# feiyeha/EGM-Unet

Hardware: AMD Instinct MI355X
Metric: train images/sec at 3x512x512 bs=8/GPU (higher is better)
Workload: dtype bf16; 1 GPU; EGM-UNet GRFBUNet(3,2,base_c=32) fwd+5-term-loss+bwd+SGD, 8x3x512x512 per GPU (BASELINE.json configs[1]); global_batch=8, parallelism=dp1, launch=hipGraph replay, world_size=1

## Files before the change

egm_unet_amd/csrc/mca.hip:

```cpp
#include "common.h"
#include "bn_elem.h"
#include <stdlib.h>

namespace {

inline int stream_grid(long long total_threads) {
    long long b = (total_threads + 255) / 256;
    if (b > 256 * 16) b = 256 * 16;
    if (b < 1) b = 1;
    return (int)b;
}
__device__ __forceinline__ float sigm(float v) { return 1.f / (1.f + expf(-v)); }

template <typename T, int MODE>
__global__ __launch_bounds__(256) void mca_reduce_row_kernel(const T* __restrict__ a, int lda, const T* __restrict__ b, int ldb,
                                                             float* __restrict__ sums, float* __restrict__ colp, float* __restrict__ chp,
                                                             int H, int W, int C, const float* __restrict__ scale = nullptr,
                                                             const float* __restrict__ shift = nullptr, int act = 0,
                                                             T* __restrict__ zout = nullptr, int ldz = 0) {
    __shared__ float st[2 * 256 * 8];
    __shared__ float red[16];
    const int n = blockIdx.y, h = blockIdx.x, tid = threadIdx.x, ncv = C >> 3, slots = 256 / ncv;
    const int cv = tid % ncv, slot = tid / ncv, L = H + W + C;
    const long long rowbase = ((long long)n * H + h) * W;
// ... 214 lines not shown
            for (int q = -1; q <= 1; ++q) {
                if (yy + r < 0 || yy + r >= H || xx + q < 0 || xx + q >= W) continue;
                load8(xo + (p + (long long)r * W + q) * ld + cv * 8, v);
#pragma unroll
                for (int j = 0; j < 8; ++j) {
                    if (v[j] > mx[j]) { mx[j] = v[j]; amx[j] = (r + 1) * 3 + (q + 1); }
                    if (v[j] < mn[j]) { mn[j] = v[j]; amn[j] = (r + 1) * 3 + (q + 1); }
                    s[j] += v[j];
                }
            }
        float o1[8], o2[8];
#pragma unroll
        for (int j = 0; j < 8; ++j) {
            const float sh = to_f32(xo[p * ld + shuffle_src(cv * 8 + j, C)]);
            o1[j] = 0.51f * c[j] + 0.2f * (mx[j] - mn[j]) + 0.1f * sh;
            const float u = c[j] - s[j] * (1.f / 9.f);
            o2[j] = u * u;
        }
        store8(r1 + p * ldr + cv * 8, o1); store8(u2 + p * ldu + cv * 8, o2);
        if (codes != nullptr) {
            uint2 cd;
            cd.x = (amx[0] | (amn[0] << 4)) | ((amx[1] | (amn[1] << 4)) << 8) | ((amx[2] | (amn[2] << 4)) << 16) | ((amx[3] | (amn[3] << 4)) << 24);
            cd.y = (amx[4] | (amn[4] << 4)) | ((amx[5] | (amn[5] << 4)) << 8) | ((amx[6] | (amn[6] << 4)) << 16) | ((amx[7] | (amn[7] << 4)) << 24);
            *reinterpret_cast<uint2*>(codes + p * C + cv * 8) = cd;
        }
    }
}
template <typename T>
__global__ void add_avg3_kernel(const T* __restrict__ a, int lda, const T* __restrict__ b, int ldb, float scale, T* __restrict__ out, int ldo,
                                int N, int H, int W, int C) {
    const int ncv = C >> 3;
    const long long total = (long long)N * H * W * ncv;
    for (long long i = blockIdx.x * 256LL + threadIdx.x; i < total; i += (long long)gridDim.x * 256) {
        long long p; int cv; egm_divmod(i, ncv, p, cv);
        int xx, yy; egm_pix_yx(p, H, W, yy, xx);
        float c[8], s[8], v[8];
        load8(a + p * lda + cv * 8, c);
        zero8(s);
#pragma unroll
        for (int r = -1; r <= 1; ++r)
#pragma unroll
            for (int q = -1; q <= 1; ++q) {
                if (yy + r < 0 || yy + r >= H || xx + q < 0 || xx + q >= W) continue;
                load8(b + (p + (long long)r * W + q) * ldb + cv * 8, v);
#pragma unroll
                for (int j = 0; j < 8; ++j) s[j] += v[j];
            }
#pragma unroll
        for (int j = 0; j < 8; ++j) c[j] += scale * s[j] * (1.f / 9.f);
        store8(out + p * ldo + cv * 8, c);
    }
}
constexpr int MF_TY = 16, MF_TX = 16, MF_CB = 32, MF_PY = MF_TY + 4, MF_PX = MF_TX + 4, MF_UY = MF_TY + 2, MF_UX = MF_TX + 2;
template <typename T>
__global__ __launch_bounds__(256) void mca_fused_fwd_kernel(const T* __restrict__ x, int ldx, const float* __restrict__ gates,
                                                            T* __restrict__ xo, int ldxo, T* __restrict__ out, int ldo,
                                                            unsigned char* __restrict__ codes, int N, int H, int W, int C, int tiles_x,
                                                            int tiles_y, int nchunk, float inv) {
    extern __shared__ __attribute__((aligned(16))) unsigned char mf_smem[];
    T* sxo = reinterpret_cast<T*>(mf_smem);
    T* su2 = sxo + MF_PY * MF_PX * MF_CB;
    const int tid = threadIdx.x, L = H + W + C;
    int b = xcd_contiguous_item(blockIdx.x, gridDim.x);
    const int chunk = b % nchunk; b /= nchunk;
    const int tx = b % tiles_x; b /= tiles_x;
    const int ty = b % tiles_y; const int n = b / tiles_y;
    const int y0 = ty * MF_TY, x0 = tx * MF_TX, c0 = chunk * MF_CB;
    const int nvec = (C - c0 < MF_CB ? C - c0 : MF_CB) >> 3;
    const float* __restrict__ g = gates + (long long)n * L;
    const long long img = (long long)n * H * W;
    __shared__ float sgh[MF_PY], sgw[MF_PX];
    if (tid < MF_PY) { const int gy = y0 + tid - 2; sgh[tid] = (gy >= 0 && gy < H) ? g[gy] : 0.f; }
    else if (tid >= 64 && tid < 64 + MF_PX) { const int gx = x0 + tid - 64 - 2; sgw[tid - 64] = (gx >= 0 && gx < W) ? g[H + gx] : 0.f; }
    const int vt = tid & 3;
    float gc8[8], gs8[8];
#pragma unroll
    for (int j = 0; j < 8; ++j) {
        const bool okv = vt < nvec;
        gc8[j] = okv ? g[H + W + c0 + vt * 8 + j] : 0.f;
        gs8[j] = okv ? g[H + W + shuffle_src(c0 + vt * 8 + j, C)] : 0.f;
    }

    constexpr int NC = MF_TY * MF_TX * 4 / 256;
    T shv[NC][8];
#pragma unroll
    for (int k = 0; k < NC; ++k) {
        const int i = tid + k * 256, pix = i >> 2, v = i & 3, ly = pix / MF_TX, lx = pix - ly * MF_TX;
        const int gy = y0 + ly, gx = x0 + lx;
        const bool ok = v < nvec && gy < H && gx < W;
        const long long p = img + (long long)(ok ? gy : 0) * W + (ok ? gx : 0);
        const int q0 = ok ? ((c0 + v * 8) >> 2) : 0;
#pragma unroll
        for (int grp = 0; grp < 4; ++grp) {
            const T* sp = x + p * ldx + (ok ? grp * (C >> 2) : 0) + q0;
            if (sizeof(T) == 2 && ((C >> 2) & 1) == 0) {
                const uint32_t two = *reinterpret_cast<const uint32_t*>(sp);
                __builtin_memcpy(&shv[k][grp], &two, 2);
                const uint16_t hi = (uint16_t)(two >> 16);
                __builtin_memcpy(&shv[k][grp + 4], &hi, 2);
            } else {
                shv[k][grp] = sp[0]; shv[k][grp + 4] = sp[1];
            }
        }
    }
    constexpr int NA = (MF_PY * MF_PX * 4 + 255) / 256;
    uint4 raw[NA];
#pragma unroll
    for (int k = 0; k < NA; ++k) {
        const int i = tid + k * 256, pix = i >> 2, v = i & 3, py = pix / MF_PX, px = pix - py * MF_PX;
        const int gy = y0 + py - 2, gx = x0 + px - 2;
        raw[k] = make_uint4(0, 0, 0, 0);
        if (i < MF_PY * MF_PX * 4 && v < nvec && gy >= 0 && gy < H && gx >= 0 && gx < W) {
            const T* src = x + (img + (long long)gy * W + gx) * ldx + c0 + v * 8;
            if (sizeof(T) == 2) raw[k] = *reinterpret_cast<const uint4*>(src);
        }
    }
    __syncthreads();
#pragma unroll
    for (int k = 0; k < NA; ++k) {
        const int i = tid + k * 256, pix = i >> 2, v = i & 3, py = pix / MF_PX, px = pix - py * MF_PX;
        const int gy = y0 + py - 2, gx = x0 + px - 2;
        if (i >= MF_PY * MF_PX * 4) continue;
        float val[8];
        zero8(val);
        if (v < nvec && gy >= 0 && gy < H && gx >= 0 && gx < W) {
            const long long p = img + (long long)gy * W + gx;
            if (sizeof(T) == 2) load8(reinterpret_cast<const T*>(&raw[k]), val);
            else load8(x + p * ldx + c0 + v * 8, val);
            const float ghw = sgh[py] + sgw[px];
#pragma unroll
            for (int j = 0; j < 8; ++j) val[j] = to_f32(from_f32<T>(val[j] * ((ghw + gc8[j]) * inv)));
            if (xo != nullptr && py >= 2 && py < MF_TY + 2 && px >= 2 && px < MF_TX + 2) store8(xo + p * ldxo + c0 + v * 8, val);
        }
        store8_lds(sxo + pix * MF_CB + v * 8, val);
    }
    __syncthreads();
    for (int i = tid; i < MF_UY * MF_UX * 4; i += 256) {
        const int pix = i >> 2, v = i & 3, uy = pix / MF_UX, ux = pix - uy * MF_UX;
        const int gy = y0 + uy - 1, gx = x0 + ux - 1;
        float o2[8];
        zero8(o2);
        if (v < nvec && gy >= 0 && gy < H && gx >= 0 && gx < W) {
            float c[8], s8[8], t[8];
            zero8(s8);
            const T* ctr = sxo + ((uy + 1) * MF_PX + ux + 1) * MF_CB + v * 8;
            load8(ctr, c);
#pragma unroll
            for (int r = -1; r <= 1; ++r)
#pragma unroll
                for (int q = -1; q <= 1; ++q) {
                    load8(ctr + (r * MF_PX + q) * MF_CB, t);
#pragma unroll
                    for (int j = 0; j < 8; ++j) s8[j] += t[j];
                }
#pragma unroll
            for (int j = 0; j < 8; ++j) { const float u = c[j] - s8[j] * (1.f / 9.f); o2[j] = u * u; }
        }
        store8_lds(su2 + pix * MF_CB + v * 8, o2);
    }
    __syncthreads();
#pragma unroll
    for (int k = 0; k < NC; ++k) {
        const int i = tid + k * 256;
        const int pix = i >> 2, v = i & 3, ly = pix / MF_TX, lx = pix - ly * MF_TX;
        const int gy = y0 + ly, gx = x0 + lx;
        if (v >= nvec || gy >= H || gx >= W) continue;
        const long long p = img + (long long)gy * W + gx;
        float c[8], mx[8], mn[8], t[8], s2[8];
        int amx[8], amn[8];
        const T* ctr = sxo + ((ly + 2) * MF_PX + lx + 2) * MF_CB + v * 8;
        const T* uctr = su2 + ((ly + 1) * MF_UX + lx + 1) * MF_CB + v * 8;
        load8(ctr, c);
        zero8(s2);
#pragma unroll
        for (int j = 0; j < 8; ++j) { mx[j] = -INFINITY; mn[j] = INFINITY; amx[j] = 4; amn[j] = 4; }
#pragma unroll
        for (int r = -1; r <= 1; ++r)
#pragma unroll
            for (int q = -1; q <= 1; ++q) {
                load8(uctr + (r * MF_UX + q) * MF_CB, t);
#pragma unroll
                for (int j = 0; j < 8; ++j) s2[j] += t[j];
                if (gy + r < 0 || gy + r >= H || gx + q < 0 || gx + q >= W) continue;
                load8(ctr + (r * MF_PX + q) * MF_CB, t);
#pragma unroll
                for (int j = 0; j < 8; ++j) {
                    if (t[j] > mx[j]) { mx[j] = t[j]; amx[j] = (r + 1) * 3 + (q + 1); }
                    if (t[j] < mn[j]) { mn[j] = t[j]; amn[j] = (r + 1) * 3 + (q + 1); }
                }
            }
        const float ghw = sgh[ly + 2] + sgw[lx + 2];
        float o[8];
#pragma unroll
        for (int j = 0; j < 8; ++j) {
            const float sh = to_f32(from_f32<T>(to_f32(shv[k][j]) * ((ghw + gs8[j]) * inv)));
            const float o1 = to_f32(from_f32<T>(0.51f * c[j] + 0.2f * (mx[j] - mn[j]) + 0.1f * sh));
            o[j] = o1 + 0.2f * s2[j] * (1.f / 9.f);
        }
        store8(out + p * ldo + c0 + v * 8, o);
        if (codes != nullptr) {
            uint2 cd;
            cd.x = (amx[0] | (amn[0] << 4)) | ((amx[1] | (amn[1] << 4)) << 8) | ((amx[2] | (amn[2] << 4)) << 16) | ((amx[3] | (amn[3] << 4)) << 24);
            cd.y = (amx[4] | (amn[4] << 4)) | ((amx[5] | (amn[5] << 4)) << 8) | ((amx[6] | (amn[6] << 4)) << 16) | ((amx[7] | (amn[7] << 4)) << 24);
            *reinterpret_cast<uint2*>(codes + p * C + c0 + v * 8) = cd;
        }
    }
}
template <typename T>
__global__ void mca_bwd_du_kernel(const T* __restrict__ xo, int ld, const T* __restrict__ g, int ldg, T* __restrict__ du, int ldd, int N, int H,
                                  int W, int C) {
    const int ncv = C >> 3;
    const long long total = (long long)N * H * W * ncv;
    for (long long i = blockIdx.x * 256LL + threadIdx.x; i < total; i += (long long)gridDim.x * 256) {
// ... 134 lines not shown
        const T* gctr = sg + ((ly + 2) * MB_P + lx + 2) * MB_CB + v * 8;
        const unsigned char* cctr = scd + ((ly + 1) * MB_U + lx + 1) * MB_CB + v * 8;
#pragma unroll
        for (int r = -1; r <= 1; ++r)
#pragma unroll
            for (int q = -1; q <= 1; ++q) {
                load8(dctr + (r * MB_U + q) * MB_CB, t);
#pragma unroll
                for (int j = 0; j < 8; ++j) sd[j] += t[j];
                load8(gctr + (r * MB_P + q) * MB_CB, gp);
                const uint2 cd = *reinterpret_cast<const uint2*>(cctr + (r * MB_U + q) * MB_CB);
                const int me = (1 - r) * 3 + (1 - q);
#pragma unroll
                for (int j = 0; j < 8; ++j) {
                    const unsigned code = ((j < 4 ? cd.x : cd.y) >> ((j & 3) * 8)) & 0xffu;
                    acc[j] += gp[j] * (((int)(code & 15u) == me ? 1.f : 0.f) - ((int)(code >> 4) == me ? 1.f : 0.f));
                }
            }
        float gc[8], dc[8], o[8];
        load8(gctr, gc); load8(dctr, dc);
#pragma unroll
        for (int j = 0; j < 8; ++j) {
            const float gs = to_f32(g[p * ldg + shuffle_dst(c0 + v * 8 + j, C)]);
            o[j] = 0.51f * gc[j] + 0.1f * gs + dc[j] - sd[j] * (1.f / 9.f) + 0.2f * acc[j];
        }
        store8(dxo + p * ldo + c0 + v * 8, o);
    }
}
template <typename T>
__global__ void mca_bwd_dx_kernel(const T* __restrict__ dxo, int ldd, const T* __restrict__ x, int ldx, const float* __restrict__ gates,
                                  const float* __restrict__ coef, T* __restrict__ dx, int ldo, int N, int H, int W, int C, float inv) {
    const int ncv = C >> 3, L = H + W + C;
    const long long total = (long long)N * H * W * ncv;
    for (long long i = blockIdx.x * 256LL + threadIdx.x; i < total; i += (long long)gridDim.x * 256) {
        long long p; int cv; egm_divmod(i, ncv, p, cv);
        int w, h, n; egm_pix_nyx(p, H, W, n, h, w);
        const float* g = gates + (long long)n * L;
        const float* cf = coef + (long long)n * L * 2;
        const float ghw = g[h] + g[H + w];
        const float A0 = cf[h * 2] + cf[(H + w) * 2], B0 = cf[h * 2 + 1] + cf[(H + w) * 2 + 1];
        float d[8], v[8];
        load8(dxo + p * ldd + cv * 8, d); load8(x + p * ldx + cv * 8, v);
#pragma unroll
        for (int j = 0; j < 8; ++j) {
            const int c = H + W + cv * 8 + j;
            d[j] = d[j] * (ghw + g[c]) * inv + (A0 + cf[c * 2]) + (B0 + cf[c * 2 + 1]) * v[j];
        }
        store8(dx + p * ldo + cv * 8, d);
    }
}

bool mca_c_ok(int C) { return C >= 8 && C <= 512 && (C & (C - 1)) == 0; }

}

#define EGM_REQ_VEC(name, ptr, ld, C)                                                                      \
    EGM_REQUIRE((ptr) != nullptr && egm_aligned16(ptr) && (C) > 0 && (C) % 8 == 0 && (ld) >= (C) && (ld) % 8 == 0, \
                name ": bad tensor (ptr/alignment/C=%d/ld=%d)", (int)(C), (int)(ld))
#define EGM_REQ_SHAPE(name) EGM_REQUIRE(N > 0 && H > 0 && W > 0, name ": bad shape")
#define EGM_MCA_GRID stream_grid((long long)N * H * W * (C / 8))

extern "C" long long egm_mca_reduce_workspace(int N, int H, int W, int C) {
    if (N <= 0 || H <= 0 || W <= 0 || !mca_c_ok(C)) return -1;
    return ((long long)N * H * W * 2 + (long long)N * H * C * 2) * 4;
}
extern "C" int egm_mca_reduce(int dtype, int mode, const void* a, int lda, const void* b, int ldb, float* sums, void* workspace, int N, int H,
                              int W, int C, egm_stream_t s) {
    EGM_REQ_VEC("mca_reduce", a, lda, C);
    if (mode == 1) EGM_REQ_VEC("mca_reduce", b, ldb, C);
    EGM_REQ_SHAPE("mca_reduce");
    EGM_REQUIRE(sums && workspace && (mode == 0 || mode == 1), "mca_reduce: bad args");
    EGM_REQUIRE(mca_c_ok(C), "mca_reduce: C must be a power of two in [8, 512] (C=%d)", C);
    float* colp = (float*)workspace;
    float* chp = colp + (long long)N * H * W * 2;
    hipStream_t st = (hipStream_t)s;
    EGM_DISPATCH_DTYPE(dtype, {
        if (mode == 0) hipLaunchKernelGGL((mca_reduce_row_kernel<T, 0>), dim3(H, N), dim3(256), 0, st, (const T*)a, lda, (const T*)b, ldb, sums,
                                          colp, chp, H, W, C);
        else hipLaunchKernelGGL((mca_reduce_row_kernel<T, 1>), dim3(H, N), dim3(256), 0, st, (const T*)a, lda, (const T*)b, ldb, sums, colp,
                                chp, H, W, C);
    });
    hipLaunchKernelGGL(mca_reduce_h_kernel, dim3(((W + C) * 2 + 15) / 16, N), dim3(256), 0, st, colp, chp, sums, N, H, W, C);
    EGM_CHECK_LAUNCH("mca_reduce");
    return EGM_OK;
}

extern "C" int egm_mca_reduce_bn(int dtype, const void* y, int ldy, const float* scale, const float* shift, int act, void* z, int ldz,
                                 float* sums, void* workspace, int N, int H, int W, int C, egm_stream_t s) {
    EGM_REQ_VEC("mca_reduce_bn", y, ldy, C);
    EGM_REQ_VEC("mca_reduce_bn", z, ldz, C);
    EGM_REQ_SHAPE("mca_reduce_bn");
    EGM_REQUIRE(sums && workspace && scale && shift, "mca_reduce_bn: bad args");
    EGM_REQUIRE(mca_c_ok(C), "mca_reduce_bn: C must be a power of two in [8, 512] (C=%d)", C);
    float* colp = (float*)workspace;
    float* chp = colp + (long long)N * H * W * 2;
    hipStream_t st = (hipStream_t)s;
    EGM_DISPATCH_DTYPE(dtype, hipLaunchKernelGGL((mca_reduce_row_kernel<T, 2>), dim3(H, N), dim3(256), 0, st, (const T*)y, ldy, (const T*)nullptr,
                                                 0, sums, colp, chp, H, W, C, scale, shift, act, (T*)z, ldz));
    hipLaunchKernelGGL(mca_reduce_h_kernel, dim3(((W + C) * 2 + 15) / 16, N), dim3(256), 0, st, colp, chp, sums, N, H, W, C);
    EGM_CHECK_LAUNCH("mca_reduce_bn");
    return EGM_OK;
}

static int gate_params(GateParams& gp, const float* w_h, const float* k_h, int ks_h, const float* w_w, const float* k_w, int ks_w,
                       const float* w_c, const float* k_c, int ks_c) {
    if (!w_h || !k_h || !w_w || !k_w || (ks_c != 0 && (!w_c || !k_c))) return 0;
// ... 17 lines not shown
}
extern "C" int egm_mca_gates_bwd(const float* dG, const float* stats, const float* o, const float* gates, const float* w_h, const float* k_h,
                                 int ks_h, const float* w_w, const float* k_w, int ks_w, const float* w_c, const float* k_c, int ks_c,
                                 float* dz_scratch, float* coef, float* dwts, float* dks, int N, int H, int W, int C, egm_stream_t s) {
    GateParams gp;
    EGM_REQUIRE(gate_params(gp, w_h, k_h, ks_h, w_w, k_w, ks_w, w_c, k_c, ks_c), "mca_gates_bwd: bad gate parameters");
    EGM_REQUIRE(dG && stats && o && gates && dz_scratch && coef && dwts && dks, "mca_gates_bwd: null pointer");
    EGM_REQ_SHAPE("mca_gates_bwd");
    const size_t lds = (size_t)4 * N * (H + W + C) * sizeof(float);
    if (lds <= 140 * 1024) {
        static bool attr_done = false;
        if (!attr_done) {
            hipError_t e = hipFuncSetAttribute(reinterpret_cast<const void*>(mca_gates_bwd_kernel<true>), hipFuncAttributeMaxDynamicSharedMemorySize, 140 * 1024);
            if (e != hipSuccess) EGM_FAIL(EGM_ERR_LAUNCH, "mca_gates_bwd: hipFuncSetAttribute: %s", hipGetErrorString(e));
            attr_done = true;
        }
        hipLaunchKernelGGL(mca_gates_bwd_kernel<true>, dim3(1), dim3(1024), lds, (hipStream_t)s, dG, stats, o, gates, gp, dz_scratch, coef, dwts, dks, N,
                           H, W, C);
    } else {
        hipLaunchKernelGGL(mca_gates_bwd_kernel<false>, dim3(1), dim3(1024), 0, (hipStream_t)s, dG, stats, o, gates, gp, dz_scratch, coef, dwts, dks, N,
                           H, W, C);
    }
    EGM_CHECK_LAUNCH("mca_gates_bwd");
    return EGM_OK;
}
extern "C" int egm_mca_xout(int dtype, const void* x, int ldx, const float* gates, void* xo, int ldo, int N, int H, int W, int C,
                            int no_spatial, egm_stream_t s) {
    const float inv = no_spatial ? 0.5f : 1.f / 3.f;
    EGM_REQ_VEC("mca_xout", x, ldx, C); EGM_REQ_VEC("mca_xout", xo, ldo, C); EGM_REQ_SHAPE("mca_xout");
    EGM_REQUIRE(gates, "mca_xout: null gates");
    EGM_DISPATCH_DTYPE(dtype, hipLaunchKernelGGL((mca_xout_kernel<T>), dim3(EGM_MCA_GRID), dim3(256), 0, (hipStream_t)s, (const T*)x, ldx, gates,
                                                 (T*)xo, ldo, N, H, W, C, inv));
    EGM_CHECK_LAUNCH("mca_xout");
    return EGM_OK;
}
extern "C" int egm_mca_stencil1(int dtype, const void* xo, int ld, void* r1, int ldr, void* u2, int ldu, unsigned char* codes, int N, int H,
                                int W, int C, egm_stream_t s) {
    EGM_REQ_VEC("mca_stencil1", xo, ld, C); EGM_REQ_VEC("mca_stencil1", r1, ldr, C); EGM_REQ_VEC("mca_stencil1", u2, ldu, C);
    EGM_REQ_SHAPE("mca_stencil1");
    EGM_REQUIRE(C % 4 == 0 && (codes == nullptr || (reinterpret_cast<uintptr_t>(codes) & 7) == 0), "mca_stencil1: bad codes buffer");
    EGM_DISPATCH_DTYPE(dtype, hipLaunchKernelGGL((mca_stencil1_kernel<T>), dim3(EGM_MCA_GRID), dim3(256), 0, (hipStream_t)s, (const T*)xo, ld,
                                                 (T*)r1, ldr, (T*)u2, ldu, codes, N, H, W, C));
    EGM_CHECK_LAUNCH("mca_stencil1");
    return EGM_OK;
}
extern "C" int egm_add_avg3(int dtype, const void* a, int lda, const void* b, int ldb, float scale, void* out, int ldo, int N, int H, int W,
                            int C, egm_stream_t s) {
    EGM_REQ_VEC("add_avg3", a, lda, C); EGM_REQ_VEC("add_avg3", b, ldb, C); EGM_REQ_VEC("add_avg3", out, ldo, C); EGM_REQ_SHAPE("add_avg3");
    EGM_DISPATCH_DTYPE(dtype, hipLaunchKernelGGL((add_avg3_kernel<T>), dim3(EGM_MCA_GRID), dim3(256), 0, (hipStream_t)s, (const T*)a, lda,
                                                 (const T*)b, ldb, scale, (T*)out, ldo, N, H, W, C));
    EGM_CHECK_LAUNCH("add_avg3");
    return EGM_OK;
}
template <typename T>
static int launch_mca_fused(const void* x, int ldx, const float* gates, void* xo, int ldxo, void* out, int ldo, unsigned char* codes, int N, int H,
                            int W, int C, float inv, hipStream_t st) {
    const size_t smem = (size_t)(MF_PY * MF_PX + MF_UY * MF_UX) * MF_CB * sizeof(T);
    static bool attr_done = false;
    if (!attr_done) {
        hipError_t e = hipFuncSetAttribute(reinterpret_cast<const void*>(mca_fused_fwd_kernel<T>), hipFuncAttributeMaxDynamicSharedMemorySize,
                                           (int)smem);
        if (e != hipSuccess) EGM_FAIL(EGM_ERR_LAUNCH, "mca_fused_fwd: hipFuncSetAttribute: %s", hipGetErrorString(e));
        attr_done = true;
    }
    const int tiles_x = (W + MF_TX - 1) / MF_TX, tiles_y = (H + MF_TY - 1) / MF_TY, nchunk = (C + MF_CB - 1) / MF_CB;
    const long long grid = (long long)N * tiles_x * tiles_y * nchunk;
    EGM_REQUIRE(grid < (1LL << 31), "mca_fused_fwd: grid too large");
    hipLaunchKernelGGL((mca_fused_fwd_kernel<T>), dim3((unsigned)grid), dim3(256), smem, st, (const T*)x, ldx, gates, (T*)xo, ldxo, (T*)out, ldo,
                       codes, N, H, W, C, tiles_x, tiles_y, nchunk, inv);
    EGM_CHECK_LAUNCH("mca_fused_fwd");
    return EGM_OK;
}
extern "C" int egm_mca_fused_fwd(int dtype, const void* x, int ldx, const float* gates, void* xo, int ldxo, void* out, int ldo,
                                 unsigned char* codes, int N, int H, int W, int C, int no_spatial, egm_stream_t s) {
    const float inv = no_spatial ? 0.5f : 1.f / 3.f;
    EGM_REQ_VEC("mca_fused_fwd", x, ldx, C); EGM_REQ_VEC("mca_fused_fwd", out, ldo, C); EGM_REQ_SHAPE("mca_fused_fwd");
    if (xo != nullptr) EGM_REQ_VEC("mca_fused_fwd", xo, ldxo, C);
    EGM_REQUIRE(gates && C % 4 == 0 && (codes == nullptr || (reinterpret_cast<uintptr_t>(codes) & 7) == 0), "mca_fused_fwd: bad gates / codes buffer");
    if (dtype == EGM_BF16) return launch_mca_fused<bf16_t>(x, ldx, gates, xo, ldxo, out, ldo, codes, N, H, W, C, inv, (hipStream_t)s);
    if (dtype == EGM_F32) return launch_mca_fused<float>(x, ldx, gates, xo, ldxo, out, ldo, codes, N, H, W, C, inv, (hipStream_t)s);
    EGM_FAIL(EGM_ERR_ARG, "mca_fused_fwd: unknown dtype %d", dtype);
}
extern "C" int egm_mca_bwd_du(int dtype, const void* xo, int ld, const void* g, int ldg, void* du, int ldd, int N, int H, int W, int C,
                              egm_stream_t s) {
    EGM_REQ_VEC("mca_bwd_du", xo, ld, C); EGM_REQ_VEC("mca_bwd_du", g, ldg, C); EGM_REQ_VEC("mca_bwd_du", du, ldd, C); EGM_REQ_SHAPE("mca_bwd_du");
    EGM_DISPATCH_DTYPE(dtype, hipLaunchKernelGGL((mca_bwd_du_kernel<T>), dim3(EGM_MCA_GRID), dim3(256), 0, (hipStream_t)s, (const T*)xo, ld,
                                                 (const T*)g, ldg, (T*)du, ldd, N, H, W, C));
    EGM_CHECK_LAUNCH("mca_bwd_du");
    return EGM_OK;
}
extern "C" int egm_mca_bwd_dxo(int dtype, const unsigned char* codes, const void* g, int ldg, const void* du, int ldd, void* dxo, int ldo,
                               int N, int H, int W, int C, egm_stream_t s) {
    EGM_REQ_VEC("mca_bwd_dxo", g, ldg, C); EGM_REQ_VEC("mca_bwd_dxo", du, ldd, C); EGM_REQ_VEC("mca_bwd_dxo", dxo, ldo, C);
    EGM_REQ_SHAPE("mca_bwd_dxo");
    EGM_REQUIRE(codes && (reinterpret_cast<uintptr_t>(codes) & 7) == 0 && C % 4 == 0, "mca_bwd_dxo: bad codes buffer");
    EGM_DISPATCH_DTYPE(dtype, hipLaunchKernelGGL((mca_bwd_dxo_kernel<T>), dim3(EGM_MCA_GRID), dim3(256), 0, (hipStream_t)s, codes, (const T*)g,
                                                 ldg, (const T*)du, ldd, (T*)dxo, ldo, N, H, W, C));
    EGM_CHECK_LAUNCH("mca_bwd_dxo");
    return EGM_OK;
}
extern "C" int egm_mca_bwd_dudxo(int dtype, const unsigned char* codes, const void* xo, int ldxo, const void* g, int ldg, void* dxo, int ldo,
                                 int N, int H, int W, int C, egm_stream_t s) {
    EGM_REQ_VEC("mca_bwd_dudxo", xo, ldxo, C); EGM_REQ_VEC("mca_bwd_dudxo", g, ldg, C); EGM_REQ_VEC("mca_bwd_dudxo", dxo, ldo, C);
    EGM_REQ_SHAPE("mca_bwd_dudxo");
    EGM_REQUIRE(codes && (reinterpret_cast<uintptr_t>(codes) & 7) == 0 && C % 4 == 0, "mca_bwd_dudxo: bad codes buffer");
    if (dtype != EGM_BF16) EGM_FAIL(EGM_ERR_UNSUPPORTED, "mca_bwd_dudxo: bf16 only (fp32: egm_mca_bwd_du + egm_mca_bwd_dxo)");
    const int tiles_x = (W + MB_T - 1) / MB_T, tiles_y = (H + MB_T - 1) / MB_T, nchunk = (C + MB_CB - 1) / MB_CB;
    const long long grid = (long long)N * tiles_x * tiles_y * nchunk;
    EGM_REQUIRE(grid < (1LL << 31), "mca_bwd_dudxo: grid too large");
    hipLaunchKernelGGL((mca_bwd_fused_kernel<bf16_t>), dim3((unsigned)grid), dim3(256), 0, (hipStream_t)s, codes, (const bf16_t*)xo, ldxo,
                       (const bf16_t*)g, ldg, (bf16_t*)dxo, ldo, N, H, W, C, tiles_x, tiles_y, nchunk);
    EGM_CHECK_LAUNCH("mca_bwd_dudxo");
    return EGM_OK;
}
extern "C" int egm_mca_bwd_dx(int dtype, const void* dxo, int ldd, const void* x, int ldx, const float* gates, const float* coef, void* dx,
                              int ldo, int N, int H, int W, int C, int no_spatial, egm_stream_t s) {
    const float inv = no_spatial ? 0.5f : 1.f / 3.f;
    EGM_REQ_VEC("mca_bwd_dx", dxo, ldd, C); EGM_REQ_VEC("mca_bwd_dx", x, ldx, C); EGM_REQ_VEC("mca_bwd_dx", dx, ldo, C);
    EGM_REQ_SHAPE("mca_bwd_dx");
    EGM_REQUIRE(gates && coef, "mca_bwd_dx: null pointer");
    EGM_DISPATCH_DTYPE(dtype, hipLaunchKernelGGL((mca_bwd_dx_kernel<T>), dim3(EGM_MCA_GRID), dim3(256), 0, (hipStream_t)s, (const T*)dxo, ldd,
                                                 (const T*)x, ldx, gates, coef, (T*)dx, ldo, N, H, W, C, inv));
    EGM_CHECK_LAUNCH("mca_bwd_dx");
    return EGM_OK;
}
```

include/egm_hip.h:

```cpp
#ifndef EGM_HIP_H
#define EGM_HIP_H

#ifdef __cplusplus
extern "C" {
#endif

typedef void* egm_stream_t;

enum egm_status { EGM_OK = 0, EGM_ERR_ARG = -1, EGM_ERR_LAUNCH = -2, EGM_ERR_UNSUPPORTED = -3 };
enum egm_dtype { EGM_F32 = 0, EGM_BF16 = 1 };
enum egm_act { EGM_ACT_NONE = 0, EGM_ACT_RELU = 1, EGM_ACT_SIGMOID = 2, EGM_ACT_SILU = 3  };

int egm_version(void);
const char* egm_last_error(void);
int egm_device_ok(void);

int egm_nchw_to_nhwc(int dtype, const void* src_f32, void* dst, int ld, int N, int C, int H, int W, egm_stream_t s);
int egm_nhwc_to_nchw(int dtype, const void* src, int ld, void* dst_f32, int N, int C, int H, int W, egm_stream_t s);

int egm_conv_pack(int dtype, const void* w_oihw_f32, void* wf, void* wd, int Cout, int Cin, int KH, int KW, int groups,
                  egm_stream_t s);
int egm_conv_pack_chunk(void);
int egm_conv_pack_multi(int dtype, const void* table_dev, int n, long long total_chunks, egm_stream_t s);
int egm_group_begin(void);
// ... 202 lines not shown
int egm_sa_conv7_bwd(int dtype, const void* x, int ldx, const void* dy, int lddy, const float* w, void* dx, int lddx, float* dw,
                     void* workspace, int N, int H, int W, egm_stream_t s);
long long egm_global_pool_workspace(int N, long long HW, int C);
int egm_global_avgmax_fwd(int dtype, const void* x, int ldx, void* out, int* argidx, void* workspace, int N, long long HW,
                          int C, egm_stream_t s);
int egm_global_avgmax_bwd(int dtype, const void* gout, const int* argidx, void* dx, int lddx, int N, long long HW, int C,
                          egm_stream_t s);
int egm_rows_dup(int dtype, const float* red, void* dst, int ldd, int N, int C, egm_stream_t s);
int egm_ca_mlp_fwd(int dtype, const void* pooled, int ldp, const float* w0, const float* w2, float* h, void* logits, int ldo, int R,
                   int C, int Cr, egm_stream_t s);
int egm_ca_mlp_bwd(int dtype, const void* dlogits, int ldd, const void* pooled, int ldp, const float* h, const float* w0,
                   const float* w2, float* dw0, float* dw2, void* dpooled, int lddp, int R, int C, int Cr, egm_stream_t s);
int egm_fusion_combine_fwd(int dtype, const void* f, int ldf, const void* sv, int lds, const void* sa, int ldsa, const void* ca,
                           void* out, int ldo, int N, long long HW, int C, egm_stream_t s);
int egm_fusion_combine_blocks(long long HW, int C);
int egm_fusion_combine_bwd(int dtype, const void* g, int ldg, const void* sv, int lds, const void* sa, int ldsa, const void* ca,
                           void* ds, int ldds, void* dsa, int lddsa, float* partials, int N, long long HW, int C, egm_stream_t s);
int egm_fold2_fwd(const float* w, float* out, int rows, int K, egm_stream_t s);
int egm_fold2_bwd(const float* g, float* dw, int rows, int K, egm_stream_t s);
int egm_merge357_fwd(const float* w3, const float* w5, const float* w7, const float* b3, const float* b5, const float* b7,
                     float* w, float* b, int Co, int Ci, egm_stream_t s);
int egm_merge357_bwd(const float* gw, float* d3, float* d5, float* d7, const float* gb, float* gb3, int Co, int Ci, egm_stream_t s);
int egm_fold2_pack(int dtype, const float* w, float* out, void* wf, void* wd, int rows, int K, egm_stream_t s);
int egm_merge357_pack(int dtype, const float* w3, const float* w5, const float* w7, const float* b3, const float* b5, const float* b7,
                      float* w, float* b, void* wf, void* wd, int Co, int Ci, egm_stream_t s);

long long egm_mca_reduce_workspace(int N, int H, int W, int C);
int egm_mca_reduce(int dtype, int mode, const void* a, int lda, const void* b, int ldb, float* sums, void* workspace, int N,
                   int H, int W, int C, egm_stream_t s);
int egm_mca_reduce_bn(int dtype, const void* y, int ldy, const float* scale, const float* shift, int act, void* z, int ldz,
                      float* sums, void* workspace, int N, int H, int W, int C, egm_stream_t s);
int egm_mca_gates_fwd(const float* sums, const float* w_h, const float* k_h, int ks_h, const float* w_w, const float* k_w,
                      int ks_w, const float* w_c, const float* k_c, int ks_c, float* stats, float* o, float* gates, int N, int H,
                      int W, int C, egm_stream_t s);
int egm_mca_gates_bwd(const float* dG, const float* stats, const float* o, const float* gates, const float* w_h, const float* k_h,
                      int ks_h, const float* w_w, const float* k_w, int ks_w, const float* w_c, const float* k_c, int ks_c,
                      float* dz_scratch, float* coef, float* dwts, float* dks, int N, int H, int W, int C, egm_stream_t s);
int egm_mca_xout(int dtype, const void* x, int ldx, const float* gates, void* xo, int ldo, int N, int H, int W, int C,
                 int no_spatial, egm_stream_t s);
int egm_mca_stencil1(int dtype, const void* xo, int ld, void* r1, int ldr, void* u2, int ldu, unsigned char* codes, int N, int H,
                     int W, int C, egm_stream_t s);
int egm_add_avg3(int dtype, const void* a, int lda, const void* b, int ldb, float scale, void* out, int ldo, int N, int H, int W,
                 int C, egm_stream_t s);
int egm_mca_fused_fwd(int dtype, const void* x, int ldx, const float* gates, void* xo, int ldxo, void* out, int ldo, unsigned char* codes,
                      int N, int H, int W, int C, int no_spatial, egm_stream_t s);
int egm_mca_bwd_du(int dtype, const void* xo, int ld, const void* g, int ldg, void* du, int ldd, int N, int H, int W, int C,
                   egm_stream_t s);
int egm_mca_bwd_dxo(int dtype, const unsigned char* codes, const void* g, int ldg, const void* du, int ldd, void* dxo, int ldo,
                    int N, int H, int W, int C, egm_stream_t s);
int egm_mca_bwd_dudxo(int dtype, const unsigned char* codes, const void* xo, int ldxo, const void* g, int ldg, void* dxo, int ldo,
                      int N, int H, int W, int C, egm_stream_t s);
int egm_mca_bwd_dx(int dtype, const void* dxo, int ldd, const void* x, int ldx, const float* gates, const float* coef, void* dx,
                   int ldo, int N, int H, int W, int C, int no_spatial, egm_stream_t s);

int egm_gemm(int dtype, const void* A, int lda, const void* B, int ldb, int transB, void* C, int ldc, int c_is_f32,
             const float* bias, int act, const void* R, int ldr, float alpha, int M, int N, int K, int nb1, int nb2,
             long long sA1, long long sA2, long long sB1, long long sB2, long long sC1, long long sC2, long long sR1,
             long long sR2, egm_stream_t s);
int egm_gemm_dma_mode(int mode);
int egm_attention_fused(int dtype, const void* qkv, int ld, int B, int L, int H, int head_dim, int mode, void* out, int ldo,
                        egm_stream_t s);
int egm_softmax_rows(int dtype, const float* S, int lds, void* P, int ldp, long long rows, int L, int causal, int accumulate,
                     egm_stream_t s);
int egm_layernorm(int dtype, const void* x, int ldx, const float* gamma, const float* beta, float eps, void* y, int ldy,
                  long long rows, int D, egm_stream_t s);
int egm_patchify(int dtype, const float* img_nchw, void* out, int B, int C, int H, int W, int P, egm_stream_t s);
int egm_vit_assemble(int dtype, const void* tok, const float* cls, const float* pos, void* x, int B, int Ltok, int D, egm_stream_t s);
int egm_text_embed(int dtype, const int* tokens, const float* emb, const float* pos, const float* pos_res, int split, void* x,
                   int n, int L, int D, egm_stream_t s);
int egm_film(int dtype, void* a, const void* mul, const void* add, int B, int L, int D, egm_stream_t s);
int egm_gather_rows(int dtype, const void* x, const int* idx, void* out, int n, int L, int D, egm_stream_t s);
int egm_pixel_shuffle(int dtype, const void* y, int ldy, int tok_off, int Ltot, const float* bias, float* out, int B, int g,
                      int P, egm_stream_t s);
int egm_cast_f32(int dtype, const float* src, void* dst, long long n, egm_stream_t s);

long long egm_loss_workspace(int N, int C);
int egm_loss_fwd(const float* logits, const long long* target, const float* class_weight, int N, int C, int H, int W,
                 long long ignore_index, int dice, float* loss6, float* workspace, unsigned char* signs, egm_stream_t s);
int egm_loss_bwd(const float* logits, const long long* target, const float* class_weight, int N, int C, int H, int W,
                 long long ignore_index, int dice, const float* workspace, const unsigned char* signs, const float* grad_out,
                 float* dlogits, egm_stream_t s);
int egm_argmax_hist(const float* logits, const long long* target, int N, int C, int H, int W, long long dice_ignore_index,
                    unsigned long long* hist, unsigned long long* counts, long long* pred, egm_stream_t s);
int egm_metrics_finalize(const unsigned long long* hist, const unsigned long long* counts, int N, int C, float* out,
                         egm_stream_t s);
int egm_ensemble_fuse(const float* clip_logits, const float* unet_logits, float alpha, int N, int C, int hc, int wc, int H, int W,
                      long long* pred, float* fused, egm_stream_t s);
int egm_ensemble_alpha_hist(const float* clip_logits, const float* unet_logits, const long long* target, const float* alphas, int na,
                            int N, int C, int hc, int wc, int H, int W, unsigned long long* hist, egm_stream_t s);
int egm_ensemble_miou(const unsigned long long* hist, int na, int C, float* miou, egm_stream_t s);
int egm_sgd_chunk(void);
int egm_sgd_multi(const void* table_dev, int ntensors, long long total_chunks, const float* lr_dev, float lr, float momentum,
                  float weight_decay, float grad_scale, int first_step, egm_stream_t s);
int egm_copy_multi(const void* table_dev, int ntensors, egm_stream_t s);

int egm_convT2x2_pack(float* w_iohw, float* w4, int Cin, int Cout, int CoutP, int to_packed, egm_stream_t s);
int egm_shuffle2x2_fwd(int dtype, const void* y4, int ld4, const float* bias, int bias_n, void* out, int ldo, int N, int H, int W, int C,
                       int Ho, int Wo, int oy, int ox, egm_stream_t s);
int egm_shuffle2x2_bwd(int dtype, const void* g, int ldg, void* d4, int ld4, int N, int H, int W, int C, int Ho, int Wo, int oy, int ox,
                       egm_stream_t s);

int egm_ela_strip_means(int dtype, const void* x, int ldx, float* mh, float* mw, int N, int H, int W, int C, egm_stream_t s);
int egm_ela_gates_fwd(const float* mh, const float* mw, const float* conv_w, int ks, const float* gamma, const float* beta, float eps,
                      float* yh, float* yw, float* gh, float* gw, float* stats, int N, int H, int W, int C, int groups, egm_stream_t s);
int egm_ela_apply(int dtype, const void* x, int ldx, const float* gh, const float* gw, void* out, int ldo, int N, int H, int W, int C,
                  egm_stream_t s);
// ... 151 lines not shown
```

Measured before the change: 686.5 images/s.

## Add strip-based register-reuse path to fused MCA forward stencil kernel

Adds a STRIPS variant of the fused MCA forward kernel, enabled by default for bf16 and switchable through EGM_MCA_MODE. Each thread walks a vertical strip of rows and keeps sliding 3x3 windows in registers, so the box-average, max/min and argmax stencils no longer reload nine neighbours from LDS for every output pixel. It also unpacks bf16 with bit shifts and writes packed outputs and codes directly. The cost is higher register pressure, some idle threads in phase B, and a more complex edge-handling path that has to reproduce the old argmax codes exactly.

```diff
diff --git a/egm_unet_amd/csrc/mca.hip b/egm_unet_amd/csrc/mca.hip
--- a/egm_unet_amd/csrc/mca.hip
+++ b/egm_unet_amd/csrc/mca.hip
@@ -290,7 +290,17 @@
     }
 }
 constexpr int MF_TY = 16, MF_TX = 16, MF_CB = 32, MF_PY = MF_TY + 4, MF_PX = MF_TX + 4, MF_UY = MF_TY + 2, MF_UX = MF_TX + 2;
-template <typename T>
+__device__ __forceinline__ float bf16x8_ch(const uint4& a, int j) {
+    const uint32_t w = (j >> 1) == 0 ? a.x : ((j >> 1) == 1 ? a.y : ((j >> 1) == 2 ? a.z : a.w));
+    return __uint_as_float((j & 1) ? (w & 0xffff0000u) : (w << 16));
+}
+__device__ __forceinline__ float bf16x4_ch(const uint2& a, int j) {
+    const uint32_t w = (j >> 1) == 0 ? a.x : a.y;
+    return __uint_as_float((j & 1) ? (w & 0xffff0000u) : (w << 16));
+}
+__device__ __forceinline__ float scan_first_max(float v) { float r; asm("v_max_f32 %0, 0xff800000, %1" : "=v"(r) : "v"(v)); return r; }
+__device__ __forceinline__ float scan_first_min(float v) { float r; asm("v_min_f32 %0, 0x7f800000, %1" : "=v"(r) : "v"(v)); return r; }
+template <typename T, bool STRIPS>
 __global__ __launch_bounds__(256) void mca_fused_fwd_kernel(const T* __restrict__ x, int ldx, const float* __restrict__ gates,
                                                             T* __restrict__ xo, int ldxo, T* __restrict__ out, int ldo,
                                                             unsigned char* __restrict__ codes, int N, int H, int W, int C, int tiles_x,
@@ -321,9 +331,10 @@
 
     constexpr int NC = MF_TY * MF_TX * 4 / 256;
     T shv[NC][8];
+    uint32_t shw[NC][4];
 #pragma unroll
     for (int k = 0; k < NC; ++k) {
-        const int i = tid + k * 256, pix = i >> 2, v = i & 3, ly = pix / MF_TX, lx = pix - ly * MF_TX;
+        const int i = tid + k * 256, pix = i >> 2, v = i & 3, ly = STRIPS ? (tid >> 6) * NC + k : pix / MF_TX, lx = pix - (pix / MF_TX) * MF_TX;
         const int gy = y0 + ly, gx = x0 + lx;
         const bool ok = v < nvec && gy < H && gx < W;
         const long long p = img + (long long)(ok ? gy : 0) * W + (ok ? gx : 0);
@@ -331,7 +342,9 @@
 #pragma unroll
         for (int grp = 0; grp < 4; ++grp) {
             const T* sp = x + p * ldx + (ok ? grp * (C >> 2) : 0) + q0;
-            if (sizeof(T) == 2 && ((C >> 2) & 1) == 0) {
+            if constexpr (STRIPS) {
+                shw[k][grp] = *reinterpret_cast<const uint32_t*>(sp);
+            } else if (sizeof(T) == 2 && ((C >> 2) & 1) == 0) {
                 const uint32_t two = *reinterpret_cast<const uint32_t*>(sp);
                 __builtin_memcpy(&shv[k][grp], &two, 2);
                 const uint16_t hi = (uint16_t)(two >> 16);
@@ -373,6 +386,46 @@
         store8_lds(sxo + pix * MF_CB + v * 8, val);
     }
     __syncthreads();
+    if constexpr (STRIPS) {
+        constexpr int SB = 6;
+        static_assert(MF_UY % SB == 0 && MF_UX * 4 * (MF_UY / SB) <= 256, "phase B strips");
+        if (tid < MF_UX * 4 * (MF_UY / SB)) {
+            const int v = tid & 3, ux = (tid >> 2) % MF_UX, uy0 = (tid / (MF_UX * 4)) * SB;
+            const int gx = x0 + ux - 1;
+            const bool okc = v < nvec && gx >= 0 && gx < W;
+            const uint4* prow = reinterpret_cast<const uint4*>(sxo + (uy0 * MF_PX + ux) * MF_CB + v * 8);
+            constexpr int PIX4 = MF_CB * 2 / 16;
+            uint4 a[SB + 2][3];
+#pragma unroll
+            for (int r = 0; r < 2; ++r)
+#pragma unroll
+                for (int q = 0; q < 3; ++q) a[r][q] = prow[(r * MF_PX + q) * PIX4];
+#pragma unroll
+            for (int k = 0; k < SB; ++k) {
+                const int gy = y0 + uy0 + k - 1;
+#pragma unroll
+                for (int q = 0; q < 3; ++q) a[k + 2][q] = prow[((k + 2) * MF_PX + q) * PIX4];
+                float o2[8];
+#pragma unroll
+                for (int j = 0; j < 8; ++j) {
+                    float s = 0.f;
+#pragma unroll
+                    for (int r = 0; r < 3; ++r)
+#pragma unroll
+                        for (int q = 0; q < 3; ++q) s += bf16x8_ch(a[k + r][q], j);
+                    const float u = __builtin_fmaf(-s, 1.f / 9.f, bf16x8_ch(a[k + 1][1], j));
+                    o2[j] = u * u;
+                }
+                const uint32_t keep = (okc && gy >= 0 && gy < H) ? 0xffffffffu : 0u;
+                uint4 pk;
+                pk.x = ((uint32_t)f32_to_bf16(o2[0]) | ((uint32_t)f32_to_bf16(o2[1]) << 16)) & keep;
+                pk.y = ((uint32_t)f32_to_bf16(o2[2]) | ((uint32_t)f32_to_bf16(o2[3]) << 16)) & keep;
+                pk.z = ((uint32_t)f32_to_bf16(o2[4]) | ((uint32_t)f32_to_bf16(o2[5]) << 16)) & keep;
+                pk.w = ((uint32_t)f32_to_bf16(o2[6]) | ((uint32_t)f32_to_bf16(o2[7]) << 16)) & keep;
+                *reinterpret_cast<uint4*>(su2 + ((uy0 + k) * MF_UX + ux) * MF_CB + v * 8) = pk;
+            }
+        }
+    } else
     for (int i = tid; i < MF_UY * MF_UX * 4; i += 256) {
         const int pix = i >> 2, v = i & 3, uy = pix / MF_UX, ux = pix - uy * MF_UX;
         const int gy = y0 + uy - 1, gx = x0 + ux - 1;
@@ -397,6 +450,94 @@
         store8_lds(su2 + pix * MF_CB + v * 8, o2);
     }
     __syncthreads();
+    if constexpr (STRIPS) {
+        const int v = tid & 3, lx = (tid >> 2) & (MF_TX - 1), ly0 = (tid >> 6) * NC;
+        const int gx = x0 + lx, gy0 = y0 + ly0;
+        if (v < nvec && gx < W && gy0 < H) {
+            const int ql = gx > 0 ? 0 : 1, qr = gx + 1 < W ? 2 : 1;
+            constexpr int PIX2 = MF_CB * 2 / 8;
+            const float gwx = sgw[lx + 2];
+            const int top = gy0 > 0 ? 0 : 1, hlim = H - gy0;
+            uint32_t ow[NC][2], cw[NC];
+#pragma unroll 1
+            for (int h = 0; h < 2; ++h) {
+                float gsh[4];
+#pragma unroll
+                for (int j = 0; j < 4; ++j) gsh[j] = h ? gs8[4 + j] : gs8[j];
+                const int shl = h ? 0 : 16;
+                const uint2* xrow = reinterpret_cast<const uint2*>(sxo + ((ly0 + 1) * MF_PX + lx + 1) * MF_CB + v * 8 + h * 4);
+                const uint2* urow = reinterpret_cast<const uint2*>(su2 + (ly0 * MF_UX + lx) * MF_CB + v * 8 + h * 4);
+                float mx[NC][4], mn[NC][4], s2[NC][4];
+                int amx[NC][4], amn[NC][4];
+                uint2 ctr[NC];
+#pragma unroll
+                for (int i = 0; i < NC + 2; ++i) {
+                    {
+                        const uint2 u0 = urow[(i * MF_UX + 0) * PIX2], u1 = urow[(i * MF_UX + 1) * PIX2], u2v = urow[(i * MF_UX + 2) * PIX2];
+#pragma unroll
+                        for (int k = (i >= 2 ? i - 2 : 0); k <= (i < NC ? i : NC - 1); ++k)
+#pragma unroll
+                            for (int j = 0; j < 4; ++j) {
+                                float s = (k == i) ? 0.f : s2[k][j];
+                                s += bf16x4_ch(u0, j); s += bf16x4_ch(u1, j); s += bf16x4_ch(u2v, j);
+                                s2[k][j] = s;
+                            }
+                    }
+                    const int ri = i == 0 ? top : (i < hlim ? i : hlim);
+                    const uint2* xr = xrow + ri * (MF_PX * PIX2);
+                    const uint2 a0 = xr[ql * PIX2], a1 = xr[PIX2], a2 = xr[qr * PIX2];
+                    if (i >= 1 && i <= NC) ctr[i - 1] = a1;
+#pragma unroll
+                    for (int j = 0; j < 4; ++j) {
+                        const float f0 = bf16x4_ch(a0, j), f1 = bf16x4_ch(a1, j), f2 = bf16x4_ch(a2, j);
+                        float rmx = scan_first_max(f0), rmn = scan_first_min(f0);
+                        int rcx = ql, rcn = ql;
+                        if (f1 > rmx) { rmx = f1; rcx = 1; }
+                        if (f1 < rmn) { rmn = f1; rcn = 1; }
+                        if (f2 > rmx) { rmx = f2; rcx = 2; }
+                        if (f2 < rmn) { rmn = f2; rcn = 2; }
+#pragma unroll
+                        for (int k = (i >= 2 ? i - 2 : 0); k <= (i < NC ? i : NC - 1); ++k) {
+                            const int r = i - k;
+                            if (r == 0) {
+                                const int roff = i == 0 ? 3 * top : 0;
+                                mx[k][j] = rmx; amx[k][j] = rmx > -INFINITY ? rcx + roff : 4;
+                                mn[k][j] = rmn; amn[k][j] = rmn < INFINITY ? rcn + roff : 4;
+                            } else {
+                                if (rmx > mx[k][j]) { mx[k][j] = rmx; amx[k][j] = rcx + 3 * r; }
+                                if (rmn < mn[k][j]) { mn[k][j] = rmn; amn[k][j] = rcn + 3 * r; }
+                            }
+                        }
+                    }
+                    if (i >= 2) {
+                        const int k = i - 2;
+                        const float ghw = sgh[ly0 + k + 2] + gwx;
+                        float o[4];
+#pragma unroll
+                        for (int j = 0; j < 4; ++j) {
+                            const float shx = __uint_as_float((shw[k][j] << shl) & 0xffff0000u);
+                            const float sh = to_f32(from_f32<T>(shx * ((ghw + gsh[j]) * inv)));
+                            const float c = bf16x4_ch(ctr[k], j);
+                            const float o1 = to_f32(from_f32<T>(__builtin_fmaf(0.1f, sh, __builtin_fmaf(0.51f, c, 0.2f * (mx[k][j] - mn[k][j])))));
+                            o[j] = __builtin_fmaf(0.2f * s2[k][j], 1.f / 9.f, o1);
+                        }
+                        const uint32_t w0 = (uint32_t)f32_to_bf16(o[0]) | ((uint32_t)f32_to_bf16(o[1]) << 16);
+                        const uint32_t w1 = (uint32_t)f32_to_bf16(o[2]) | ((uint32_t)f32_to_bf16(o[3]) << 16);
+                        const uint32_t cd = (amx[k][0] | (amn[k][0] << 4)) | ((amx[k][1] | (amn[k][1] << 4)) << 8) | ((amx[k][2] | (amn[k][2] << 4)) << 16) | ((amx[k][3] | (amn[k][3] << 4)) << 24);
+                        if (h == 0) {
+                            ow[k][0] = w0; ow[k][1] = w1; cw[k] = cd;
+                        } else if (gy0 + k < H) {
+                            const long long p = img + (long long)(gy0 + k) * W + gx;
+                            egm_u32x4 a;
+                            a.x = ow[k][0]; a.y = ow[k][1]; a.z = w0; a.w = w1;
+                            egm_store16_as<EGM_STORE_MODE>(out + p * ldo + c0 + v * 8, a);
+                            if (codes != nullptr) *reinterpret_cast<uint2*>(codes + p * C + c0 + v * 8) = make_uint2(cw[k], cd);
+                        }
+                    }
+                }
+            }
+        }
+    } else
 #pragma unroll
     for (int k = 0; k < NC; ++k) {
         const int i = tid + k * 256;
@@ -637,6 +778,15 @@
 
 bool mca_c_ok(int C) { return C >= 8 && C <= 512 && (C & (C - 1)) == 0; }
 
+int g_mca_mode = -1;
+
+}
+
+extern "C" int egm_mca_mode(int mode) {
+    if (g_mca_mode < 0) g_mca_mode = getenv("EGM_MCA_MODE") ? atoi(getenv("EGM_MCA_MODE")) : 1;
+    const int old = g_mca_mode;
+    if (mode >= 0) g_mca_mode = mode;
+    return old;
 }
 
 #define EGM_REQ_VEC(name, ptr, ld, C)                                                                      \
@@ -760,13 +910,13 @@
     EGM_CHECK_LAUNCH("add_avg3");
     return EGM_OK;
 }
-template <typename T>
+template <typename T, bool STRIPS>
 static int launch_mca_fused(const void* x, int ldx, const float* gates, void* xo, int ldxo, void* out, int ldo, unsigned char* codes, int N, int H,
                             int W, int C, float inv, hipStream_t st) {
     const size_t smem = (size_t)(MF_PY * MF_PX + MF_UY * MF_UX) * MF_CB * sizeof(T);
     static bool attr_done = false;
     if (!attr_done) {
-        hipError_t e = hipFuncSetAttribute(reinterpret_cast<const void*>(mca_fused_fwd_kernel<T>), hipFuncAttributeMaxDynamicSharedMemorySize,
+        hipError_t e = hipFuncSetAttribute(reinterpret_cast<const void*>(mca_fused_fwd_kernel<T, STRIPS>), hipFuncAttributeMaxDynamicSharedMemorySize,
                                            (int)smem);
         if (e != hipSuccess) EGM_FAIL(EGM_ERR_LAUNCH, "mca_fused_fwd: hipFuncSetAttribute: %s", hipGetErrorString(e));
         attr_done = true;
@@ -774,7 +924,7 @@
     const int tiles_x = (W + MF_TX - 1) / MF_TX, tiles_y = (H + MF_TY - 1) / MF_TY, nchunk = (C + MF_CB - 1) / MF_CB;
     const long long grid = (long long)N * tiles_x * tiles_y * nchunk;
     EGM_REQUIRE(grid < (1LL << 31), "mca_fused_fwd: grid too large");
-    hipLaunchKernelGGL((mca_fused_fwd_kernel<T>), dim3((unsigned)grid), dim3(256), smem, st, (const T*)x, ldx, gates, (T*)xo, ldxo, (T*)out, ldo,
+    hipLaunchKernelGGL((mca_fused_fwd_kernel<T, STRIPS>), dim3((unsigned)grid), dim3(256), smem, st, (const T*)x, ldx, gates, (T*)xo, ldxo, (T*)out, ldo,
                        codes, N, H, W, C, tiles_x, tiles_y, nchunk, inv);
     EGM_CHECK_LAUNCH("mca_fused_fwd");
     return EGM_OK;
@@ -785,8 +935,10 @@
     EGM_REQ_VEC("mca_fused_fwd", x, ldx, C); EGM_REQ_VEC("mca_fused_fwd", out, ldo, C); EGM_REQ_SHAPE("mca_fused_fwd");
     if (xo != nullptr) EGM_REQ_VEC("mca_fused_fwd", xo, ldxo, C);
     EGM_REQUIRE(gates && C % 4 == 0 && (codes == nullptr || (reinterpret_cast<uintptr_t>(codes) & 7) == 0), "mca_fused_fwd: bad gates / codes buffer");
-    if (dtype == EGM_BF16) return launch_mca_fused<bf16_t>(x, ldx, gates, xo, ldxo, out, ldo, codes, N, H, W, C, inv, (hipStream_t)s);
-    if (dtype == EGM_F32) return launch_mca_fused<float>(x, ldx, gates, xo, ldxo, out, ldo, codes, N, H, W, C, inv, (hipStream_t)s);
+    if (dtype == EGM_BF16 && egm_mca_mode(-1) != 0)
+        return launch_mca_fused<bf16_t, true>(x, ldx, gates, xo, ldxo, out, ldo, codes, N, H, W, C, inv, (hipStream_t)s);
+    if (dtype == EGM_BF16) return launch_mca_fused<bf16_t, false>(x, ldx, gates, xo, ldxo, out, ldo, codes, N, H, W, C, inv, (hipStream_t)s);
+    if (dtype == EGM_F32) return launch_mca_fused<float, false>(x, ldx, gates, xo, ldxo, out, ldo, codes, N, H, W, C, inv, (hipStream_t)s);
     EGM_FAIL(EGM_ERR_ARG, "mca_fused_fwd: unknown dtype %d", dtype);
 }
 extern "C" int egm_mca_bwd_du(int dtype, const void* xo, int ld, const void* g, int ldg, void* du, int ldd, int N, int H, int W, int C,
diff --git a/include/egm_hip.h b/include/egm_hip.h
--- a/include/egm_hip.h
+++ b/include/egm_hip.h
@@ -278,6 +278,7 @@
                       int N, int H, int W, int C, egm_stream_t s);
 int egm_mca_bwd_dx(int dtype, const void* dxo, int ldd, const void* x, int ldx, const float* gates, const float* coef, void* dx,
                    int ldo, int N, int H, int W, int C, int no_spatial, egm_stream_t s);
+int egm_mca_mode(int mode);
 
 int egm_gemm(int dtype, const void* A, int lda, const void* B, int ldb, int transB, void* C, int ldc, int c_is_f32,
              const float* bias, int act, const void* R, int ldr, float alpha, int M, int N, int K, int nb1, int nb2,
```

Result: no change. 692.4 images/s (median of 6 runs) (+0.9%).
